# YuePanEdward/MULLS

Hardware: NVIDIA H100
Metric: scan-pair registrations/sec (120k-pt 64-beam) (higher is better)
Workload: dtype f32 geometry / f64 accumulation

## Files before the change

### mulls_b200/csrc/device_types.cuh

```cuda
#pragma once
#include <cstdint>
#include <cuda_runtime.h>

#include "../../include/mulls_b200/abi.h"
#include "search_core.cuh"

namespace mulls {

constexpr int kNumClasses = MULLS_NUM_CLASSES;
constexpr int kNumSegs = 2 * kNumClasses;
constexpr int kIterBlock = 128;
constexpr int kIngestBlock = 256;
constexpr int kTerms = 28;
constexpr int kMaxLevels = 12;
constexpr int kCoordBits = 12;
constexpr int kDedupMinSrc = 500;
constexpr unsigned kClaimFree = 0x7f7f7f7fu;
constexpr int kIterFlags = 256;

enum PairStatus : int { kRunning = 0, kNeedPosterior = 1, kDone = 2 };

struct ChunkDesc {
    uint32_t pair;
    uint32_t seg;
// ... 37 lines not shown
};

struct PairState {
    double T_total[16];
    double T_inc[16];
    double x[6];
    double cofactor[36];
    double info[36];
    double sigma2;
    double ibb[6];
    float thre;
    float confidence;
    float origin[3];
    float h0, inv_h0;
    int n_levels;
    int status, code, iter, iters_entered, final_buf;
    int source_feature_points_count;
    int n_src[kNumClasses];
    int n_src_g[kNumClasses];
    int n_src_g_next[kNumClasses];
    int n_tgt[kNumClasses];
    uint32_t n_corr[kNumClasses];
    uint32_t n_corr_last[kNumClasses];
    uint32_t seg_count[kNumSegs];
    uint32_t seg_start[kNumSegs];
    uint32_t hash_entries[kNumClasses];
    uint32_t hash_base[kNumClasses];
    uint32_t hash_mask[kNumClasses];
    int bb_src[6];
    int bb_tgt[6];
    uint64_t alg_bytes;
    int kl_keep[kNumSegs];
    uint32_t kl_rank[kNumSegs];
    uint64_t kl_prefix[kNumSegs];
    uint32_t kl_hist[kNumSegs][256];
};

struct LoopCtl {
    int it;
    int n_it_chunks;
    int n_pairs;
    int trace_on;
    int max_iter;
    unsigned solved;
    unsigned n_live[2];
    unsigned work[4];
};

struct DeviceArrays {
    const float4 *in_aos;
    uint64_t *keys_a, *keys_b;
    uint32_t *vals_a, *vals_b;
    float4 *tgt_pos, *tgt_nrm;
    float4 *src_pos[2], *src_nrm[2];
    int *src_prevj[2];
    float4 *src_cert[2];
    int *nn_idx;
    float *nn_d2;
    uint8_t *flags;
    int *corr_j;
    float *corr_w;
    unsigned *claim;
    HashEntry *hash;
    uint32_t hash_pool_entries;
    uint32_t *hash_used;
    uint32_t *blk_kept;
    double *partials;
    double *post_partials;
    PairConst *pc;
    PairState *ps;
    ChunkDesc *in_chunks;
    ChunkDesc *it_chunks;
    mulls_icp_trace *trace;
    int *xch_i32;
    double *xch_f64;
    LoopCtl *ctl;
    uint32_t *live_chunks;
    uint32_t live_stride;
    int *running;
    volatile int *h_running;
    volatile int *h_running_iter;
};

}
```

### mulls_b200/csrc/kernels_iterate.cuh

```cuda
#pragma once
#include <cooperative_groups.h>

#include "device_math.cuh"
#include "device_types.cuh"
#include "kernels_ingest.cuh"

namespace mulls {

__device__ __forceinline__ bool chunk_in_run(const DeviceArrays &A) { return blockIdx.x < (unsigned)A.ctl->n_it_chunks; }
__device__ __forceinline__ int loop_buf(const DeviceArrays &A, int buf) { return buf >= 0 ? buf : (A.ctl->it & 1); }
__device__ __forceinline__ mulls_icp_trace *trace_of(const DeviceArrays &A, uint32_t pair) {
    return (A.trace && A.ctl->trace_on) ? &A.trace[pair] : nullptr;
}

template <class Body>
__device__ __forceinline__ void for_each_live_chunk(const DeviceArrays &A, int parity, int which, Body body) {
    __shared__ uint32_t s_fetch;
    LoopCtl &ctl = *A.ctl;
    const uint32_t n = ctl.n_live[parity];
    const uint32_t *list = A.live_chunks + (size_t)parity * A.live_stride;
    for (;;) {
        __syncthreads();
        if (threadIdx.x == 0) s_fetch = atomicAdd(&ctl.work[which], 1u);
        __syncthreads();
// ... 26 lines not shown
}

constexpr int kStartLevel0 = 5;
constexpr int kLeafCount = 32;
constexpr int kDeferFromIter = 3;
constexpr float kReseedCells = 4.0f;

__device__ __forceinline__ GridView grid_of(const DeviceArrays &A, const PairConst &pc, const PairState &ps, int c) {
    GridView g;
    g.table = A.hash + ps.hash_base[c];
    g.mask = ps.hash_mask[c];
    g.pos = A.tgt_pos + pc.tgt_base[c];
    g.nrm = A.tgt_nrm + pc.tgt_base[c];
    g.ox = ps.origin[0], g.oy = ps.origin[1], g.oz = ps.origin[2];
    g.h0 = ps.h0, g.inv_h0 = ps.inv_h0;
    g.n_levels = ps.n_levels;
    g.leaf_count = kLeafCount;
    g.level_slack2 = 1.002001f;
    return g;
}

constexpr int kShootK = 10;

__device__ __forceinline__ void load_and_advance(DeviceArrays &A, const PairState &ps, int buf, uint32_t gi, bool valid,
                                                 float4 &p, float4 &n) {
    p = A.src_pos[buf][gi];
    n = A.src_nrm[buf][gi];
    if (valid && ps.iter > 0) {
        const double *t = ps.T_inc;
        const double px = p.x, py = p.y, pz = p.z, qx = n.x, qy = n.y, qz = n.z;
        p.x = (float)(t[0] * px + t[1] * py + t[2] * pz + t[3]);
        p.y = (float)(t[4] * px + t[5] * py + t[6] * pz + t[7]);
        p.z = (float)(t[8] * px + t[9] * py + t[10] * pz + t[11]);
        n.x = (float)(t[0] * qx + t[1] * qy + t[2] * qz);
        n.y = (float)(t[4] * qx + t[5] * qy + t[6] * qz);
        n.z = (float)(t[8] * qx + t[9] * qy + t[10] * qz);
        A.src_pos[buf][gi] = p;
        A.src_nrm[buf][gi] = n;
    }
}

__device__ __forceinline__ bool shoots(const PairConst &pc, int c) {
    return pc.normal_shooting && (c == MULLS_GROUND || c == MULLS_FACADE || c == MULLS_ROOF);
}

constexpr int kKeepFromIter = 3;

struct SearchFrame {
    GridView g;
    double max_dist_sqr;
    float r2_prune;
    bool defer;
};
__device__ __forceinline__ SearchFrame search_frame(const DeviceArrays &A, const PairConst &pc, const PairState &ps, int c) {
    SearchFrame f;
    f.g = grid_of(A, pc, ps, c);
    const float max_distance_f = 2.5f * ps.thre;
    f.max_dist_sqr = (double)max_distance_f * (double)max_distance_f;
    f.r2_prune = (float)f.max_dist_sqr * 1.0001f;
    f.defer = ps.iter >= kDeferFromIter;
    return f;
// ... 89 lines not shown
                need = true;
                const int pj = A.src_prevj[buf][gi];
                const float4 ce = A.src_cert[buf][gi];
                if (pj >= 0 && ce.w > 0.0f) {
                    const float4 q = __ldg(&f.g.pos[pj]);
                    const float d1 = flann_l2(p.x, p.y, p.z, q.x, q.y, q.z);
                    const float mv = flann_l2(p.x, p.y, p.z, ce.x, ce.y, ce.z);
                    if ((sqrtf(d1) + sqrtf(mv)) * 1.0001f + 3e-5f < ce.w * 0.9999f) {
                        search_finish(A, pc, c, gi, pj, d1, f.max_dist_sqr, n.w);
                        need = false;
                    }
                }
            }
        }
        const unsigned m = __ballot_sync(0xffffffffu, need);
        uint32_t base = 0;
        if (lane == 0 && m) base = atomicAdd(n_need, (uint32_t)__popc(m));
        base = __shfl_sync(0xffffffffu, base, 0);
        if (need) need_list[base + __popc(m & ((1u << lane) - 1u))] = (uint8_t)threadIdx.x;
    }
    __syncthreads();
    if (threadIdx.x < *n_need) {
        const uint32_t gi = pc.src_base[c] + cd.first + need_list[threadIdx.x];
        const float4 p = A.src_pos[buf][gi];
        search_one<WalkBounds>(A, pc, c, buf, gi, p, A.src_nrm[buf][gi].w, f, true);
    }
}

constexpr int kSearchBlocksPerSm = 10;
__device__ __forceinline__ int search_mode_of(int it) { return it >= kKeepFromIter ? 2 : (it == kKeepFromIter - 1 ? 1 : 0); }

template <int kMode>
__global__ void __launch_bounds__(kIterBlock, kSearchBlocksPerSm) k_search(DeviceArrays A, int buf, int it) {
    buf = loop_buf(A, buf);
    if (it < 0) it = A.ctl->it;
    if (blockIdx.x == 0 && threadIdx.x == 0) {
        LoopCtl &ctl = *A.ctl;
        ctl.work[1] = ctl.work[2] = ctl.work[3] = 0u;
        ctl.n_live[buf ^ 1] = 0u;
    }
    if (search_mode_of(it) != kMode) return;
    if (kMode == 2) {
        __shared__ uint8_t s_need[kIterBlock];
        __shared__ uint32_t s_n_need;
        for_each_live_chunk(A, buf, 0, [&](uint32_t chunk) { search_keep_chunk(A, buf, chunk, s_need, &s_n_need); });
    } else {
        const uint32_t n_units = (kIterBlock / 32) * A.ctl->n_live[buf];
// ... 36 lines not shown
    KnnList<kShootK> kl;
    knn_search(g, p.x, p.y, p.z, kStartLevel0, kShootK, kl);
    double min_dist = 1.7976931348623157e308;
    for (int t = 0; t < kl.n; ++t) {
        const float4 q = __ldg(&g.pos[kl.j[t]]);
        const float ptx = q.x - p.x, pty = q.y - p.y, ptz = q.z - p.z;
        const double Nx = n.x, Ny = n.y, Nz = n.z, Vx = ptx, Vy = pty, Vz = ptz;
        const double Cx = Ny * Vz - Nz * Vy, Cy = Nz * Vx - Nx * Vz, Cz = Nx * Vy - Ny * Vx;
        const double dist = Cx * Cx + (Cy * Cy + Cz * Cz);
        if (dist < min_dist) {
            min_dist = dist;
            sj = kl.j[t];
            sd2 = kl.d2[t];
        }
    }
    if (sj >= 0 && min_dist > (double)max_distance_f) sj = -1;
    if (sj >= 0) atomicMin(&A.claim[pc.tgt_base[c] + sj], (unsigned)__float_as_int(n.w));
    A.nn_idx[gi] = sj;
    A.nn_d2[gi] = sd2;
}
__global__ void __launch_bounds__(kIterBlock) k_search_shoot(DeviceArrays A, int buf) {
    buf = loop_buf(A, buf);
    for_each_live_chunk(A, buf, 3, [&](uint32_t chunk) { search_shoot_chunk(A, buf, chunk); });
}

__device__ __forceinline__ void resolve_body(DeviceArrays &A, int buf, uint32_t chunk) {
    const ChunkDesc cd = A.it_chunks[chunk];
    const PairConst &pc = A.pc[cd.pair];
    PairState &ps = A.ps[cd.pair];
    if (ps.status != kRunning) return;
    const int c = (int)cd.seg;
    const int ns = ps.n_src[c], nt = ps.n_tgt[c], nsg = ps.n_src_g[c];
    const uint32_t local = cd.first + threadIdx.x;
    const bool valid = (int)local < ns;
    const bool active = pc.used[c] && nsg >= 3 && nt >= 3;
    const bool dedup = active && nsg >= kDedupMinSrc;
    bool kept = false, pass = false;
    if (valid) {
        const uint32_t gi = pc.src_base[c] + local;
        const int j = A.nn_idx[gi];
        const bool matched = active && j >= 0;
        bool corr = matched;
        kept = true;
        if (dedup) {
            const float4 n = A.src_nrm[buf][gi];
            const bool winner = matched && A.claim[pc.tgt_base[c] + j] == (unsigned)__float_as_int(n.w);
            kept = winner;
            corr = winner;
        }
        if (corr) {
            const float d2 = A.nn_d2[gi];
            pass = d2 < ps.thre * ps.thre;
            if (pass && c != MULLS_VERTEX) {
                const float4 n = A.src_nrm[buf][gi];
                const float4 m = A.tgt_nrm[pc.tgt_base[c] + j];
                const double dot = (double)n.x * (double)m.x + (double)n.y * (double)m.y + (double)n.z * (double)m.z;
                const float cos_angle = (float)fabs(dot);
                if ((double)cos_angle < pc.cos_thre) pass = false;
            }
        }
        A.flags[gi] = (uint8_t)((kept ? 1 : 0) | (pass ? 2 : 0));
    }
    const unsigned kb = __ballot_sync(0xffffffffu, kept);
    const unsigned pb = __ballot_sync(0xffffffffu, pass);
    __shared__ unsigned s_kept[kIterBlock / 32], s_pass[kIterBlock / 32];
    if ((threadIdx.x & 31) == 0) {
        s_kept[threadIdx.x >> 5] = __popc(kb);
        s_pass[threadIdx.x >> 5] = __popc(pb);
    }
    __syncthreads();
    if (threadIdx.x == 0) {
        unsigned k = 0, p = 0;
        for (int w = 0; w < kIterBlock / 32; ++w) {
            k += s_kept[w];
            p += s_pass[w];
        }
        A.blk_kept[chunk] = k;
        if (p) atomicAdd(&ps.n_corr[c], p);
    }
}
__global__ void __launch_bounds__(kIterBlock) k_resolve(DeviceArrays A, int buf) {
    buf = loop_buf(A, buf);
    for_each_live_chunk(A, buf, 1, [&](uint32_t chunk) { resolve_body(A, buf, chunk); });
}

template <class Sink>
__device__ __forceinline__ void terms_pt2pl(const float4 p, const float pi, const float4 q, const float4 qn,
                                            float weight, int iter_num, bool dist_w, bool resid_w, bool inten_w,
                                            float window, Sink t, float &w_out) {
    const float px = p.x, py = p.y, pz = p.z, qx = q.x, qy = q.y, qz = q.z;
    const float ntx = qn.x, nty = qn.y, ntz = qn.z;
    float w = weight;
    const float a = ntz * py - nty * pz;
    const float b = ntx * pz - ntz * px;
    const float c = nty * px - ntx * py;
    const float d = ntx * qx + nty * qy + ntz * qz - ntx * px - nty * py - ntz * pz;
    const float dist = sqrtf(qx * qx + qy * qy + qz * qz);
    if (dist_w) w = w * weight_by_dist_adaptive(dist, iter_num);
    if (resid_w) w = w * weight_by_residual(fabsf(d), window);
    if (inten_w) w = w * weight_by_intensity((float)((double)pi + 0.0001), (float)((double)q.w + 0.0001));
    w_out = w;
    t[0] = w * ntx * ntx;
    t[1] = w * ntx * nty;
    t[2] = w * ntx * ntz;
// ... 242 lines not shown
                cof[6 * (3 + r) + cc] = J[r][0] * inv[6 * 3 + cc] + J[r][1] * inv[6 * 4 + cc] + J[r][2] * inv[6 * 5 + cc];
    }
    double *Tt = ps.T_inc;
    construct_trans_a(x, Tt);
    const double ts_norm = sqrt(Tt[3] * Tt[3] + Tt[7] * Tt[7] + Tt[11] * Tt[11]);
    const double rs_angle = fabs(rotation_angle(Tt));
    if (ts_norm > (double)pc.max_t || rs_angle > (double)pc.max_r) {
        ps.code = -1;
        ps.status = kDone;
        pair_left_running(A);
        return;
    }
    mat4_mul(Tt, ps.T_total, Tmp);
    for (int k = 0; k < 16; ++k) ps.T_total[k] = Tmp[k];
    if (i == pc.max_iter - 1 || (i > 2 && ts_norm < (double)pc.conv_t && rs_angle < (double)pc.conv_r)) {
        ps.status = kNeedPosterior;
        ps.final_buf = buf_written;
        pair_left_running(A);
        return;
    }
    ps.iter = i + 1;
}

__device__ __forceinline__ void accumulate_body(DeviceArrays &A, int buf, uint32_t chunk) {
    const ChunkDesc cd = A.it_chunks[chunk];
    const PairConst &pc = A.pc[cd.pair];
    PairState &ps = A.ps[cd.pair];
    if (ps.status != kRunning) return;
    const int c = (int)cd.seg;
    const int ns = ps.n_src[c];
    const uint32_t local = cd.first + threadIdx.x;
    const bool valid = (int)local < ns;
    const int lane = threadIdx.x & 31, warp = threadIdx.x >> 5;
    constexpr int kWarps = kIterBlock / 32;
    __shared__ double s_terms[27 * kIterBlock];
    __shared__ uint32_t s_off[kWarps + 1];
    __shared__ uint32_t s_base;

    if ((int)cd.first >= ns) return;
    uint32_t dst_local = 0;
    uint8_t fl = 0;
    uint32_t gi = 0;
    bool kept = false, pass = false;
    struct Column {
        double *base;
        __device__ __forceinline__ double &operator[](int k) const { return base[k * kIterBlock]; }
    } t = {s_terms + threadIdx.x};
    {
        uint32_t acc = 0;
        const uint32_t first_chunk = pc.class_chunk_begin[c];
        for (uint32_t b = first_chunk + threadIdx.x; b < chunk; b += kIterBlock) acc += A.blk_kept[b];
        for (int o = 16; o > 0; o >>= 1) acc += __shfl_xor_sync(0xffffffffu, acc, o);
        if (lane == 0) s_off[warp] = acc;
        __syncthreads();
        if (threadIdx.x == 0) {
            uint32_t tt = 0;
            for (int w = 0; w < kWarps; ++w) tt += s_off[w];
            s_base = tt;
        }
        __syncthreads();
    }
    if (valid) {
        gi = pc.src_base[c] + local;
        fl = A.flags[gi];
    }
    kept = (fl & 1) != 0, pass = (fl & 2) != 0;
    const unsigned kb = __ballot_sync(0xffffffffu, kept);
    if (lane == 0) s_off[warp] = __popc(kb);
    __syncthreads();
    if (threadIdx.x == 0) {
        uint32_t run = 0;
        for (int w = 0; w < kWarps; ++w) {
            const uint32_t tt = s_off[w];
            s_off[w] = run;
            run += tt;
        }
        s_off[kWarps] = run;
    }
    __syncthreads();
    dst_local = s_base + s_off[warp] + __popc(kb & ((1u << lane) - 1u));

    float w_store = 0.0f;
    int j = -1;
    float4 p = make_float4(0, 0, 0, 0), n = make_float4(0, 0, 0, 0);
    float d2 = 0.0f;
    if (valid) {
        p = A.src_pos[buf][gi];
        n = A.src_nrm[buf][gi];
        j = A.nn_idx[gi];
        d2 = A.nn_d2[gi];
        if (j >= 0) A.claim[pc.tgt_base[c] + j] = kClaimFree;
    }
    uint32_t n_corr[kNumClasses];
#pragma unroll
    for (int k = 0; k < kNumClasses; ++k) n_corr[k] = ps.n_corr[k];
    float ratio_unused;
    const bool few = too_few(pc, ps, n_corr, ratio_unused);
    if (pass && !few) {
        const float4 q = A.tgt_pos[pc.tgt_base[c] + j];
        const float4 qn = A.tgt_nrm[pc.tgt_base[c] + j];
        const int it = ps.iter;
        const bool resid_w = pc.w_residual && it > 2;
        const bool dist_w = pc.w_dist != 0, inten_w = pc.w_intensity != 0;
        if (c == MULLS_GROUND || c == MULLS_FACADE || c == MULLS_ROOF) {
            const float wc = (c == MULLS_FACADE) ? 1.0f : balanced_ground_weight(pc, n_corr);
            terms_pt2pl(p, p.w, q, qn, wc, it, dist_w, resid_w, inten_w, pc.win_pt2pl, t, w_store);
        } else if (c == MULLS_PILLAR || c == MULLS_BEAM) {
            terms_pt2li(p, p.w, q, qn, 1.0f, it, dist_w, resid_w, inten_w, pc.win_pt2li, t, w_store);
        } else {
            terms_pt2pt(p, p.w, q, 1.0f, it, dist_w, resid_w, inten_w, pc.win_pt2pt, t);
            w_store = d2;
        }
    } else {
#pragma unroll
        for (int k = 0; k < 27; ++k) t[k] = 0.0;
    }
    if (kept) {
        const uint32_t gd = pc.src_base[c] + dst_local;
        A.src_pos[buf ^ 1][gd] = p;
        A.src_nrm[buf ^ 1][gd] = n;
        A.src_prevj[buf ^ 1][gd] = j;
        A.src_cert[buf ^ 1][gd] = A.src_cert[buf][gi];
        A.corr_j[gd] = pass ? j : -1;
        A.corr_w[gd] = w_store;
    }
    __syncthreads();
#pragma unroll 1
    for (int k = warp; k < 27; k += kWarps) {
        const double *row = s_terms + k * kIterBlock;
        double v = ((row[lane] + row[lane + 32]) + row[lane + 64]) + row[lane + 96];
#pragma unroll
        for (int o = 16; o > 0; o >>= 1) v += __shfl_xor_sync(0xffffffffu, v, o);
        if (lane == 0) A.partials[(size_t)chunk * kTerms + k] = v;
    }
}
__global__ void __launch_bounds__(kIterBlock, 8) k_accumulate(DeviceArrays A, int buf) {
    buf = loop_buf(A, buf);
    if (blockIdx.x == 0 && threadIdx.x == 0) A.ctl->work[0] = 0u;
    for_each_live_chunk(A, buf, 2, [&](uint32_t chunk) { accumulate_body(A, buf, chunk); });
}

__device__ __forceinline__ void publish_live_chunks(const DeviceArrays &A, uint32_t pair, int next_parity) {
    __shared__ uint32_t s_base;
    __syncthreads();
    const PairConst &pc = A.pc[pair];
    const PairState &ps = A.ps[pair];
    if (ps.status != kRunning) return;
    uint32_t count[kNumClasses], total = 0;
#pragma unroll
    for (int c = 0; c < kNumClasses; ++c) {
        count[c] = (uint32_t)((ps.n_src[c] + kIterBlock - 1) / kIterBlock);
        total += count[c];
    }
    if (threadIdx.x == 0) s_base = atomicAdd(&A.ctl->n_live[next_parity], total);
    __syncthreads();
    uint32_t base = s_base;
#pragma unroll
    for (int c = 0; c < kNumClasses; ++c) {
        append_live_chunks(A, next_parity, pc.class_chunk_begin[c], count[c], base);
        base += count[c];
    }
}

__device__ __forceinline__ void solve_body(DeviceArrays &A, int buf, uint32_t pair) {
    const PairConst &pc = A.pc[pair];
    PairState &ps = A.ps[pair];
    if (ps.status != kRunning) return;
    const int lane = threadIdx.x & 31, warp = threadIdx.x >> 5, n_warps = blockDim.x >> 5;
    __shared__ double s_S[kNumClasses][kTerms];
    __shared__ double s_scratch[160];
    __shared__ int s_newn[kNumClasses];
    __shared__ uint32_t s_ncorr[kNumClasses];
    for (int cc = warp; cc < kNumClasses; cc += n_warps) {
        const uint32_t b0 = pc.class_chunk_begin[cc];
        const uint32_t live = (uint32_t)((ps.n_src[cc] + kIterBlock - 1) / kIterBlock);
        const uint32_t b1 = min(pc.class_chunk_begin[cc + 1], b0 + live);
        double a0 = 0.0, a1 = 0.0, a2 = 0.0, a3 = 0.0;
        if (lane < 27) {
            uint32_t b = b0;
            for (; b + 4 <= b1; b += 4) {
                a0 += A.partials[(size_t)(b + 0) * kTerms + lane];
                a1 += A.partials[(size_t)(b + 1) * kTerms + lane];
                a2 += A.partials[(size_t)(b + 2) * kTerms + lane];
                a3 += A.partials[(size_t)(b + 3) * kTerms + lane];
            }
            for (; b < b1; ++b) a0 += A.partials[(size_t)b * kTerms + lane];
        }
        if (lane < kTerms) s_S[cc][lane] = (lane < 27) ? ((a0 + a1) + (a2 + a3)) : 0.0;
        uint32_t acc = 0;
        for (uint32_t b = b0 + lane; b < b1; b += 32) acc += A.blk_kept[b];
        for (int o = 16; o > 0; o >>= 1) acc += __shfl_xor_sync(0xffffffffu, acc, o);
        if (lane == 0) {
            s_newn[cc] = (int)acc;
            s_ncorr[cc] = ps.n_corr[cc];
        }
    }
    __syncthreads();
    if (threadIdx.x == 0) {
        uint64_t srcpts = 0;
        for (int cc = 0; cc < kNumClasses; ++cc)
            if (pc.used[cc]) srcpts += (uint64_t)ps.n_src_g[cc];
        ps.alg_bytes += 28ull * srcpts;
        if (pc.sharded) {
            for (int cc = 0; cc < kNumClasses; ++cc) {
                ps.n_src[cc] = s_newn[cc];
                for (int k = 0; k < kTerms; ++k) A.xch_f64[cc * kTerms + k] = (k < 27) ? s_S[cc][k] : 0.0;
            }
        } else {
        mulls_icp_trace *tr = trace_of(A, pair);
        for (int cc = 0; cc < kNumClasses; ++cc) {
            ps.n_src[cc] = s_newn[cc];
            ps.n_src_g[cc] = s_newn[cc];
            ps.n_corr[cc] = s_ncorr[cc];
            if (tr && ps.iter < MULLS_MAX_TRACE_ITERS) tr->n_src[ps.iter][cc] = (uint32_t)ps.n_src[cc];
        }
        solve_and_advance(A, pair, &s_S[0][0], s_scratch, buf ^ 1);
        for (int cc = 0; cc < kNumClasses; ++cc) ps.n_corr[cc] = 0;
        }
    }
    if (!pc.sharded) publish_live_chunks(A, pair, buf ^ 1);
}
constexpr int kSolveThreads = kNumClasses * 32;
__global__ void __launch_bounds__(kSolveThreads) k_solve(DeviceArrays A, int buf, unsigned long long loop_handle) {
    LoopCtl &ctl = *A.ctl;
    if (blockIdx.x >= (unsigned)ctl.n_pairs) return;
    solve_body(A, loop_buf(A, buf), blockIdx.x);
    if (loop_handle == 0ull) return;
    __syncthreads();
    if (threadIdx.x == 0) {
        __threadfence();
        if (atomicAdd(&ctl.solved, 1u) == (unsigned)ctl.n_pairs - 1u) {
            ctl.solved = 0;
            const int it = ctl.it + 1;
            ctl.it = it;
            __threadfence();
            const bool again = *(volatile int *)A.running > 0 && it < ctl.max_iter;
            cudaGraphSetConditional((cudaGraphConditionalHandle)loop_handle, again ? 1u : 0u);
        }
    }
}

__global__ void __launch_bounds__(kIterBlock, 4) k_icp_loop(DeviceArrays A) {
    namespace cg = cooperative_groups;
    cg::grid_group grid = cg::this_grid();
    LoopCtl &ctl = *A.ctl;
    __shared__ uint8_t s_need[kIterBlock];
    __shared__ uint32_t s_n_need;
    const int n_pairs = ctl.n_pairs, max_iter = ctl.max_iter;
    for (int it = 0; it < max_iter; ++it) {
        const int buf = it & 1;
        const uint32_t *list = A.live_chunks + (size_t)buf * A.live_stride;
        const uint32_t n_live = ctl.n_live[buf];
        if (blockIdx.x == 0 && threadIdx.x == 0) ctl.n_live[buf ^ 1] = 0u;
        for (uint32_t w = blockIdx.x; w < n_live; w += gridDim.x) {
            const uint32_t chunk = list[w];
            if (it >= kKeepFromIter) search_keep_chunk(A, buf, chunk, s_need, &s_n_need);
            else if (it == kKeepFromIter - 1) search_quarter<WalkBounds>(A, buf, chunk, threadIdx.x >> 5, true);
            else search_quarter<NoBounds>(A, buf, chunk, threadIdx.x >> 5, false);
            __syncthreads();
        }
        grid.sync();
        for (uint32_t w = blockIdx.x; w < n_live; w += gridDim.x) {
            resolve_body(A, buf, list[w]);
            __syncthreads();
        }
        grid.sync();
        for (uint32_t w = blockIdx.x; w < n_live; w += gridDim.x) {
            accumulate_body(A, buf, list[w]);
            __syncthreads();
        }
        grid.sync();
        for (int pair = blockIdx.x; pair < n_pairs; pair += gridDim.x) {
            solve_body(A, buf, (uint32_t)pair);
            __syncthreads();
        }
        grid.sync();
        if (*(volatile int *)A.running <= 0) break;
    }
}

__global__ void k_shard_pack_setup(DeviceArrays A, int phase) {
    PairState &ps = A.ps[0];
    if (phase == 0) {
        for (int d = 0; d < 3; ++d) {
            A.xch_i32[d] = ps.bb_src[d];
            A.xch_i32[3 + d] = ~ps.bb_src[3 + d];
        }
    } else if (phase == 1) {
        for (int d = 0; d < 3; ++d) {
            ps.bb_src[d] = A.xch_i32[d];
            ps.bb_src[3 + d] = ~A.xch_i32[3 + d];
        }
    } else if (phase == 2) {
        for (int c = 0; c < kNumClasses; ++c) A.xch_i32[c] = ps.n_src[c];
    } else {
        const PairConst &pc = A.pc[0];
// ... 221 lines not shown
        const GridView g = grid_of(A, pc, ps, cls);
        const float px = xyz[3 * i], py = xyz[3 * i + 1], pz = xyz[3 * i + 2];
        const float rmax = 2.5f * pc.thre_unit;
        const float r2 = rmax * rmax * 1.0001f;
        NoStats st;
        walk_greedy_seed(g, px, py, pz, kStartLevel0, best_d2, best_j, st);
        nn_search_walk(g, px, py, pz, r2, kStartLevel0, false, best_d2, best_j, st);
        if (best_j >= 0 && !((double)best_d2 <= (double)rmax * (double)rmax)) best_j = -1;
        if (best_j >= 0) best_j = __float_as_int(__ldg(&g.nrm[best_j]).w);
    }
    out_idx[i] = best_j;
    out_d2[i] = best_j >= 0 ? best_d2 : INFINITY;
}

__global__ void k_state_init(DeviceArrays A, int n_pairs) {
    const int p = blockIdx.x * blockDim.x + threadIdx.x;
    if (p >= n_pairs) return;
    PairState &ps = A.ps[p];
    for (int d = 0; d < 3; ++d) {
        ps.bb_src[d] = ps.bb_tgt[d] = 0x7fffffff;
        ps.bb_src[3 + d] = ps.bb_tgt[3 + d] = (int)0x80000000;
    }
    for (int s = 0; s < kNumSegs; ++s) ps.seg_count[s] = ps.seg_start[s] = 0;
    for (int c = 0; c < kNumClasses; ++c) ps.hash_entries[c] = ps.n_corr[c] = 0;
    ps.status = kRunning;
    if (p == 0) {
        *A.running = n_pairs;
        *A.h_running = n_pairs;
    }
}

__global__ void k_collect(DeviceArrays A, int n_pairs, mulls_icp_result *out) {
    if (n_pairs < 0) n_pairs = A.ctl->n_pairs;
    const int p = blockIdx.x * blockDim.x + threadIdx.x;
    if (p >= n_pairs) return;
    const PairState &ps = A.ps[p];
    mulls_icp_result &r = out[p];
    for (int k = 0; k < 16; ++k) r.T[k] = ps.T_total[k];
    for (int k = 0; k < 36; ++k) r.info[k] = ps.info[k];
    r.sigma = (float)sqrt(ps.sigma2);
    r.confidence = ps.confidence;
    r.code = ps.code;
    r.iters = ps.iters_entered;
    for (int c = 0; c < kNumClasses; ++c) {
        r.n_corr[c] = ps.n_corr_last[c];
        r.n_src[c] = (uint32_t)ps.n_src_g[c];
    }
// ... 5 lines not shown
```

### mulls_b200/csrc/mulls_b200.cu

```cuda
#include <algorithm>
#include <atomic>
#include <memory>
#include <cmath>
#include <cstdio>
#include <chrono>
#include <cstring>
#include <string>
#include <vector>

#include <cub/device/device_radix_sort.cuh>
#include <cub/device/device_scan.cuh>

#include <dlfcn.h>
#include <mutex>

#include "device_types.cuh"
#include "host_pack.h"
#include "scan_io.h"
#include "kernels_ingest.cuh"
#include "kernels_iterate.cuh"
#include "kernels_pca.cuh"
#include "kernels_map.cuh"
#include "kernels_classify.cuh"
#include "kernels_ground.cuh"
// ... 75 lines not shown
    void *nccl_comm = nullptr;
    bool any_keep_less = false;
    bool grid_valid = false;
    int use_graph = 1;
    cudaGraph_t graph = nullptr;
    cudaGraphExec_t graph_exec = nullptr;
    int graph_key[2] = {-1, -1};
    LoopCtl *h_ctl = nullptr;
    int num_sms = 132;
    bool any_normal_shooting = false;
    bool any_undistort = false;
    int host_pack = 2;
    float4 *h_stage = nullptr;
    size_t h_stage_slots = 0;
    cudaEvent_t ev_begin = nullptr, ev_ingest = nullptr, ev_iter = nullptr, ev_end = nullptr, ev_h2d0 = nullptr;
    bool h2d_timed = false;
    float up_ms_pack = 0.f, up_ms_host = 0.f;
    std::vector<cudaEvent_t> ev_search;
    mulls_run_stats stats{};
    std::vector<void *> allocs;
    std::string err;
    mulls_ctx *twin = nullptr;
    int loop_kernel_blocks = 0;
    struct Pending {
        uint64_t launches = 0;
        int n_search_ev = 0;
        bool graphed = false, hooked = false, active = false;
        mulls_icp_trace *trace = nullptr;
        mulls_allreduce_fn hook = nullptr;
        void *user = nullptr;
    } pend;
    Scratch pca_buf;
    Scratch cls_buf;
    Scratch gf_buf, gf_cell_buf;
    Scratch vx_buf, ext_buf;
    Scratch sor_buf;
    Scratch raw_buf;
    const mulls_map *tree_map = nullptr;
    uint64_t tree_epoch = 0;
};

#define CK(call)                                                                                      \
    do {                                                                                              \
        cudaError_t e_ = (call);                                                                      \
        if (e_ != cudaSuccess) {                                                                      \
            ctx->err = std::string(#call) + ": " + cudaGetErrorString(e_);                            \
// ... 132 lines not shown
    ALLOC(A.tgt_pos, ct + kScanOverrun);
    ALLOC(A.tgt_nrm, ct);
    for (int b = 0; b < 2; ++b) {
        ALLOC(A.src_pos[b], cs);
        ALLOC(A.src_nrm[b], cs);
        ALLOC(A.src_prevj[b], cs);
        ALLOC(A.src_cert[b], cs);
    }
    ALLOC(A.nn_idx, cs);
    ALLOC(A.nn_d2, cs);
    ALLOC(A.flags, cs);
    ALLOC(A.corr_j, cs);
    ALLOC(A.corr_w, cs);
    ALLOC(A.claim, ct);
    {
        size_t pool = 12 * ct + 64 * max_pairs * kNumClasses;
        if (pool >= (1ull << 32)) pool = (1ull << 32) - 1;
        A.hash_pool_entries = (uint32_t)pool;
        ALLOC(A.hash, pool);
    }
    ALLOC(A.hash_used, 3);
    ALLOC(A.ctl, 1);
    ALLOC(A.blk_kept, ctx->cap_it_chunks);
    ALLOC(A.partials, ctx->cap_it_chunks * kTerms);
    ALLOC(A.post_partials, ctx->cap_it_chunks * 2);
    ALLOC(A.pc, max_pairs);
    ALLOC(A.ps, max_pairs);
    ALLOC(A.in_chunks, ctx->cap_in_chunks);
    ALLOC(A.it_chunks, ctx->cap_it_chunks);
    ALLOC(A.live_chunks, 2 * ctx->cap_it_chunks);
    A.live_stride = (uint32_t)ctx->cap_it_chunks;
    {
        int sms = 0;
        if (cudaDeviceGetAttribute(&sms, cudaDevAttrMultiProcessorCount, device) != cudaSuccess || sms <= 0) sms = 132;
        ctx->num_sms = sms;
    }
    ALLOC(ctx->d_results, max_pairs + ceil_div(max_pairs * sizeof(uint64_t), sizeof(mulls_icp_result)) + 1);
    ALLOC(ctx->d_trace, max_pairs);
    ALLOC(A.running, 1);
    ALLOC(A.xch_i32, 32);
    ALLOC(A.xch_f64, kNumClasses * kTerms + 8);
#undef ALLOC
    if ((e = cudaHostAlloc((void **)&ctx->h_running, (1 + kIterFlags) * sizeof(int), cudaHostAllocMapped)) != cudaSuccess)
        return fail("mapped flag", e);
    {
        int *dptr = nullptr;
        if ((e = cudaHostGetDevicePointer((void **)&dptr, ctx->h_running, 0)) != cudaSuccess) return fail("mapped flag", e);
        A.h_running = dptr;
        A.h_running_iter = dptr + 1;
    }
    ctx->ev_done.resize(MULLS_MAX_TRACE_ITERS);
    for (auto &ev : ctx->ev_done) cudaEventCreateWithFlags(&ev, cudaEventDisableTiming);
    A.trace = ctx->d_trace;
    if ((e = cudaMallocHost((void **)&ctx->h_results, max_pairs * (sizeof(mulls_icp_result) + sizeof(uint64_t)))) != cudaSuccess)
        return fail("pinned results", e);
    if ((e = cudaMallocHost((void **)&ctx->h_flags, 3 * sizeof(uint32_t))) != cudaSuccess) return fail("pinned flags", e);
    if ((e = cudaMallocHost((void **)&ctx->h_ctl, sizeof(LoopCtl))) != cudaSuccess) return fail("pinned control block", e);
    {
// ... 423 lines not shown
    } else {
        k_hash_layout<<<1, 32, 0, st>>>(A, np);
        ++launches;
    }
    return MULLS_OK;
}

static unsigned chunk_bucket(const mulls_ctx *ctx) {
    unsigned b = 1;
    while (b < (unsigned)ctx->h_it_chunks.size()) b <<= 1;
    return b;
}
static unsigned resident_grid(const mulls_ctx *ctx, int blocks_per_sm) {
    return std::min((unsigned)(ctx->num_sms * blocks_per_sm), chunk_bucket(ctx));
}
static void launch_search(mulls_ctx *ctx, cudaStream_t st, const DeviceArrays &A, int buf, int it) {
    const unsigned grid = resident_grid(ctx, kSearchBlocksPerSm);
    const int mode = it < 0 ? -1 : (it >= kKeepFromIter ? 2 : (it == kKeepFromIter - 1 ? 1 : 0));
    if (mode < 0 || mode == 0) k_search<0><<<grid, kIterBlock, 0, st>>>(A, buf, it);
    if (mode < 0 || mode == 1) k_search<1><<<grid, kIterBlock, 0, st>>>(A, buf, it);
    if (mode < 0 || mode == 2) k_search<2><<<grid, kIterBlock, 0, st>>>(A, buf, it);
}
constexpr int kShootBlocksPerSm = 8, kResolveBlocksPerSm = 16, kAccumulateBlocksPerSm = 8;
constexpr int kPollPause = 64;

static int build_iteration_graph(mulls_ctx *ctx) {
    const int key[2] = {(int)chunk_bucket(ctx), ctx->any_normal_shooting ? 1 : 0};
    if (ctx->graph_exec && std::memcmp(key, ctx->graph_key, sizeof(key)) == 0) return MULLS_OK;
    if (ctx->graph_exec) cudaGraphExecDestroy(ctx->graph_exec), ctx->graph_exec = nullptr;
    if (ctx->graph) cudaGraphDestroy(ctx->graph), ctx->graph = nullptr;
    cudaStream_t st = ctx->stream;
    DeviceArrays A = ctx->A;
    const unsigned cap_chunks = (unsigned)std::max<size_t>(ctx->cap_it_chunks, 1), cap_pairs = (unsigned)std::max<size_t>(ctx->max_pairs, 1);
    CK(cudaGraphCreate(&ctx->graph, 0));
    cudaGraphConditionalHandle handle;
    CK(cudaGraphConditionalHandleCreate(&handle, ctx->graph, 1, cudaGraphCondAssignDefault));
    cudaGraphNodeParams wp = {cudaGraphNodeTypeConditional};
    wp.conditional.handle = handle;
    wp.conditional.type = cudaGraphCondTypeWhile;
    wp.conditional.size = 1;
    cudaGraphNode_t while_node;
    CK(cudaGraphAddNode(&while_node, ctx->graph, nullptr, 0, &wp));
    cudaGraph_t body = wp.conditional.phGraph_out[0];
    CK(cudaStreamBeginCaptureToGraph(st, body, nullptr, nullptr, 0, cudaStreamCaptureModeThreadLocal));
    launch_search(ctx, st, A, -1, -1);
    if (ctx->any_normal_shooting)
        k_search_shoot<<<resident_grid(ctx, kShootBlocksPerSm), kIterBlock, 0, st>>>(A, -1);
    k_resolve<<<resident_grid(ctx, kResolveBlocksPerSm), kIterBlock, 0, st>>>(A, -1);
    k_accumulate<<<resident_grid(ctx, kAccumulateBlocksPerSm), kIterBlock, 0, st>>>(A, -1);
    k_solve<<<cap_pairs, kSolveThreads, 0, st>>>(A, -1, (unsigned long long)handle);
    CK(cudaStreamEndCapture(st, nullptr));
    CK(cudaStreamBeginCaptureToGraph(st, ctx->graph, &while_node, nullptr, 1, cudaStreamCaptureModeThreadLocal));
    k_posterior<<<std::min(cap_chunks, chunk_bucket(ctx)), kIterBlock, 0, st>>>(A);
    k_finalize<<<(unsigned)ceil_div(cap_pairs, 64), 64, 0, st>>>(A, -1);
    k_collect<<<(unsigned)ceil_div(cap_pairs, 128), 128, 0, st>>>(A, -1, ctx->d_results);
    CK(cudaStreamEndCapture(st, nullptr));
    CK(cudaGraphInstantiate(&ctx->graph_exec, ctx->graph, 0));
    std::memcpy(ctx->graph_key, key, sizeof(key));
    return MULLS_OK;
}

static int grow_hash_pool(mulls_ctx *ctx) {
    const uint32_t need = ctx->h_flags[2];
    DeviceArrays &A = ctx->A;
    if (need <= A.hash_pool_entries || need == 0xffffffffu) {
        ctx->err = "hash pool exhausted (the target clouds need " + std::to_string(need) + " grid entries)";
        return MULLS_E_CAPACITY;
    }
    HashEntry *fresh = nullptr;
    if (cudaMalloc(&fresh, (size_t)need * sizeof(HashEntry)) != cudaSuccess) {
        cudaGetLastError();
        ctx->err = "hash pool exhausted, and no device memory to grow it to " + std::to_string(need) + " entries";
        return MULLS_E_CAPACITY;
// ... 92 lines not shown
            launch_search(ctx, st, A, buf, it);
            if (ctx->any_normal_shooting) {
                k_search_shoot<<<resident_grid(ctx, kShootBlocksPerSm), kIterBlock, 0, st>>>(A, buf);
                ++launches;
            }
            CK(cudaEventRecord(ctx->ev_search[2 * it + 1], st));
            if (hook) {
                if (hook(user, A.claim, ctx->n_tgt_total, 1, 1, (void *)st) != 0) {
                    ctx->err = "all-reduce callback failed";
                    return MULLS_E_COMM;
                }
            }
            k_resolve<<<resident_grid(ctx, kResolveBlocksPerSm), kIterBlock, 0, st>>>(A, buf);
            if (hook) {
                k_shard_counts<<<1, kIterBlock, 0, st>>>(A, 0);
                if (hook(user, A.xch_i32, 2 * kNumClasses, 1, 0, (void *)st) != 0) {
                    ctx->err = "all-reduce callback failed";
                    return MULLS_E_COMM;
                }
                k_shard_counts<<<1, kIterBlock, 0, st>>>(A, 1);
                launches += 2;
            }
            k_accumulate<<<resident_grid(ctx, kAccumulateBlocksPerSm), kIterBlock, 0, st>>>(A, buf);
            k_solve<<<(unsigned)np, kSolveThreads, 0, st>>>(A, buf, 0ull);
            if (hook) {
                if (hook(user, A.xch_f64, kNumClasses * kTerms, 0, 0, (void *)st) != 0) {
                    ctx->err = "all-reduce callback failed";
                    return MULLS_E_COMM;
                }
                k_shard_solve<<<1, 32, 0, st>>>(A, buf, std::min(it, kIterFlags - 1));
                ++launches;
            }
            CK(cudaEventRecord(ctx->ev_done[it], st));
            launches += 4;
            n_search_ev = it + 1;
        }
        k_posterior<<<n_itc, kIterBlock, 0, st>>>(A);
        if (hook) {
            k_shard_post<<<1, 32, 0, st>>>(A, 0);
            if (hook(user, A.xch_f64, 2, 0, 0, (void *)st) != 0) {
                ctx->err = "all-reduce callback failed";
                return MULLS_E_COMM;
            }
            k_shard_post<<<1, 32, 0, st>>>(A, 1);
            launches += 3;
        } else {
            k_finalize<<<(unsigned)ceil_div(np, 64), 64, 0, st>>>(A, np);
// ... 1384 lines not shown
```

Measured before the change: 6178.

## Fuse transform into consumers, precompute kept offsets, stage solve partials in shared memory

Stops writing transformed source points back in load_and_advance and instead re-applies the incremental transform at each consumer (shoot, resolve, accumulate). Resolve's last block per class now runs a block-wide scan over per-chunk kept counts, replacing accumulate's per-block prefix sum and solve's kept sum. k_solve moves to 512 threads and stages partials through dynamic shared memory with vectorised loads. The src_cert copy is skipped when the search mode does not need it. The trade is extra recomputation of the transform, a last-block atomic/threadfence pattern, and more shared memory per solve block.

```diff
diff --git a/mulls_b200/csrc/device_types.cuh b/mulls_b200/csrc/device_types.cuh
--- a/mulls_b200/csrc/device_types.cuh
+++ b/mulls_b200/csrc/device_types.cuh
@@ -83,6 +83,8 @@
     int n_tgt[kNumClasses];
     uint32_t n_corr[kNumClasses];
     uint32_t n_corr_last[kNumClasses];
+    uint32_t kept_done[kNumClasses];
+    uint32_t n_kept[kNumClasses];
     uint32_t seg_count[kNumSegs];
     uint32_t seg_start[kNumSegs];
     uint32_t hash_entries[kNumClasses];
@@ -126,6 +128,7 @@
     uint32_t hash_pool_entries;
     uint32_t *hash_used;
     uint32_t *blk_kept;
+    uint32_t *blk_off;
     double *partials;
     double *post_partials;
     PairConst *pc;
diff --git a/mulls_b200/csrc/kernels_iterate.cuh b/mulls_b200/csrc/kernels_iterate.cuh
--- a/mulls_b200/csrc/kernels_iterate.cuh
+++ b/mulls_b200/csrc/kernels_iterate.cuh
@@ -72,21 +72,31 @@
 
 constexpr int kShootK = 10;
 
-__device__ __forceinline__ void load_and_advance(DeviceArrays &A, const PairState &ps, int buf, uint32_t gi, bool valid,
+__device__ __forceinline__ void advance_pos(const PairState &ps, float4 &p) {
+    if (ps.iter > 0) {
+        const double *t = ps.T_inc;
+        const double px = p.x, py = p.y, pz = p.z;
+        p.x = (float)(t[0] * px + t[1] * py + t[2] * pz + t[3]);
+        p.y = (float)(t[4] * px + t[5] * py + t[6] * pz + t[7]);
+        p.z = (float)(t[8] * px + t[9] * py + t[10] * pz + t[11]);
+    }
+}
+__device__ __forceinline__ void advance_nrm(const PairState &ps, float4 &n) {
+    if (ps.iter > 0) {
+        const double *t = ps.T_inc;
+        const double qx = n.x, qy = n.y, qz = n.z;
+        n.x = (float)(t[0] * qx + t[1] * qy + t[2] * qz);
+        n.y = (float)(t[4] * qx + t[5] * qy + t[6] * qz);
+        n.z = (float)(t[8] * qx + t[9] * qy + t[10] * qz);
+    }
+}
+__device__ __forceinline__ void load_and_advance(const DeviceArrays &A, const PairState &ps, int buf, uint32_t gi, bool valid,
                                                  float4 &p, float4 &n) {
     p = A.src_pos[buf][gi];
     n = A.src_nrm[buf][gi];
-    if (valid && ps.iter > 0) {
-        const double *t = ps.T_inc;
-        const double px = p.x, py = p.y, pz = p.z, qx = n.x, qy = n.y, qz = n.z;
-        p.x = (float)(t[0] * px + t[1] * py + t[2] * pz + t[3]);
-        p.y = (float)(t[4] * px + t[5] * py + t[6] * pz + t[7]);
-        p.z = (float)(t[8] * px + t[9] * py + t[10] * pz + t[11]);
-        n.x = (float)(t[0] * qx + t[1] * qy + t[2] * qz);
-        n.y = (float)(t[4] * qx + t[5] * qy + t[6] * qz);
-        n.z = (float)(t[8] * qx + t[9] * qy + t[10] * qz);
-        A.src_pos[buf][gi] = p;
-        A.src_nrm[buf][gi] = n;
+    if (valid) {
+        advance_pos(ps, p);
+        advance_nrm(ps, n);
     }
 }
 
@@ -222,7 +232,8 @@
     __syncthreads();
     if (threadIdx.x < *n_need) {
         const uint32_t gi = pc.src_base[c] + cd.first + need_list[threadIdx.x];
-        const float4 p = A.src_pos[buf][gi];
+        float4 p = A.src_pos[buf][gi];
+        advance_pos(ps, p);
         search_one<WalkBounds>(A, pc, c, buf, gi, p, A.src_nrm[buf][gi].w, f, true);
     }
 }
@@ -305,6 +316,44 @@
 __global__ void __launch_bounds__(kIterBlock) k_search_shoot(DeviceArrays A, int buf) {
     buf = loop_buf(A, buf);
     for_each_live_chunk(A, buf, 3, [&](uint32_t chunk) { search_shoot_chunk(A, buf, chunk); });
+}
+
+constexpr int kScanItems = 4;
+__device__ __forceinline__ uint32_t scan_kept_offsets(const uint32_t *blk_kept, uint32_t *blk_off, uint32_t b0, uint32_t n_chunks) {
+    __shared__ uint32_t s_warp[kIterBlock / 32];
+    const int lane = threadIdx.x & 31, warp = threadIdx.x >> 5;
+    uint32_t carry = 0;
+    for (uint32_t r0 = 0; r0 < n_chunks; r0 += kIterBlock * kScanItems) {
+        const uint32_t lo = r0 + threadIdx.x * kScanItems;
+        uint32_t v[kScanItems], s = 0;
+#pragma unroll
+        for (int k = 0; k < kScanItems; ++k) {
+            v[k] = (lo + k < n_chunks) ? __ldcg(&blk_kept[b0 + lo + k]) : 0u;
+            s += v[k];
+        }
+        uint32_t incl = s;
+#pragma unroll
+        for (int o = 1; o < 32; o <<= 1) {
+            const uint32_t u = __shfl_up_sync(0xffffffffu, incl, o);
+            if (lane >= o) incl += u;
+        }
+        if (lane == 31) s_warp[warp] = incl;
+        __syncthreads();
+        uint32_t run = carry + incl - s, total = 0;
+#pragma unroll
+        for (int w = 0; w < kIterBlock / 32; ++w) {
+            if (w < warp) run += s_warp[w];
+            total += s_warp[w];
+        }
+#pragma unroll
+        for (int k = 0; k < kScanItems; ++k) {
+            if (lo + k < n_chunks) blk_off[b0 + lo + k] = run;
+            run += v[k];
+        }
+        carry += total;
+        __syncthreads();
+    }
+    return carry;
 }
 
 __device__ __forceinline__ void resolve_body(DeviceArrays &A, int buf, uint32_t chunk) {
@@ -335,7 +384,8 @@
             const float d2 = A.nn_d2[gi];
             pass = d2 < ps.thre * ps.thre;
             if (pass && c != MULLS_VERTEX) {
-                const float4 n = A.src_nrm[buf][gi];
+                float4 n = A.src_nrm[buf][gi];
+                advance_nrm(ps, n);
                 const float4 m = A.tgt_nrm[pc.tgt_base[c] + j];
                 const double dot = (double)n.x * (double)m.x + (double)n.y * (double)m.y + (double)n.z * (double)m.z;
                 const float cos_angle = (float)fabs(dot);
@@ -352,6 +402,7 @@
         s_pass[threadIdx.x >> 5] = __popc(pb);
     }
     __syncthreads();
+    __shared__ bool s_last;
     if (threadIdx.x == 0) {
         unsigned k = 0, p = 0;
         for (int w = 0; w < kIterBlock / 32; ++w) {
@@ -360,9 +411,21 @@
         }
         A.blk_kept[chunk] = k;
         if (p) atomicAdd(&ps.n_corr[c], p);
-    }
-}
-__global__ void __launch_bounds__(kIterBlock) k_resolve(DeviceArrays A, int buf) {
+        __threadfence();
+        const uint32_t n_chunks = (uint32_t)((ns + kIterBlock - 1) / kIterBlock);
+        s_last = atomicAdd(&ps.kept_done[c], 1u) == n_chunks - 1u;
+    }
+    __syncthreads();
+    if (s_last) {
+        const uint32_t total = scan_kept_offsets(A.blk_kept, A.blk_off, pc.class_chunk_begin[c],
+                                                 (uint32_t)((ns + kIterBlock - 1) / kIterBlock));
+        if (threadIdx.x == 0) {
+            ps.n_kept[c] = total;
+            ps.kept_done[c] = 0u;
+        }
+    }
+}
+__global__ void __launch_bounds__(kIterBlock, 16) k_resolve(DeviceArrays A, int buf) {
     buf = loop_buf(A, buf);
     for_each_live_chunk(A, buf, 1, [&](uint32_t chunk) { resolve_body(A, buf, chunk); });
 }
@@ -651,6 +714,12 @@
     ps.iter = i + 1;
 }
 
+__device__ __forceinline__ double *term_matrix() {
+    __shared__ __align__(16) double s_terms[27 * kIterBlock];
+    return s_terms;
+}
+constexpr uint32_t kTermMatrixChunks = (27 * kIterBlock / kTerms) & ~3u;
+
 __device__ __forceinline__ void accumulate_body(DeviceArrays &A, int buf, uint32_t chunk) {
     const ChunkDesc cd = A.it_chunks[chunk];
     const PairConst &pc = A.pc[cd.pair];
@@ -662,9 +731,8 @@
     const bool valid = (int)local < ns;
     const int lane = threadIdx.x & 31, warp = threadIdx.x >> 5;
     constexpr int kWarps = kIterBlock / 32;
-    __shared__ double s_terms[27 * kIterBlock];
+    double *s_terms = term_matrix();
     __shared__ uint32_t s_off[kWarps + 1];
-    __shared__ uint32_t s_base;
 
     if ((int)cd.first >= ns) return;
     uint32_t dst_local = 0;
@@ -675,20 +743,7 @@
         double *base;
         __device__ __forceinline__ double &operator[](int k) const { return base[k * kIterBlock]; }
     } t = {s_terms + threadIdx.x};
-    {
-        uint32_t acc = 0;
-        const uint32_t first_chunk = pc.class_chunk_begin[c];
-        for (uint32_t b = first_chunk + threadIdx.x; b < chunk; b += kIterBlock) acc += A.blk_kept[b];
-        for (int o = 16; o > 0; o >>= 1) acc += __shfl_xor_sync(0xffffffffu, acc, o);
-        if (lane == 0) s_off[warp] = acc;
-        __syncthreads();
-        if (threadIdx.x == 0) {
-            uint32_t tt = 0;
-            for (int w = 0; w < kWarps; ++w) tt += s_off[w];
-            s_base = tt;
-        }
-        __syncthreads();
-    }
+    const uint32_t s_base = A.blk_off[chunk];
     if (valid) {
         gi = pc.src_base[c] + local;
         fl = A.flags[gi];
@@ -716,6 +771,8 @@
     if (valid) {
         p = A.src_pos[buf][gi];
         n = A.src_nrm[buf][gi];
+        advance_pos(ps, p);
+        advance_nrm(ps, n);
         j = A.nn_idx[gi];
         d2 = A.nn_d2[gi];
         if (j >= 0) A.claim[pc.tgt_base[c] + j] = kClaimFree;
@@ -749,7 +806,7 @@
         A.src_pos[buf ^ 1][gd] = p;
         A.src_nrm[buf ^ 1][gd] = n;
         A.src_prevj[buf ^ 1][gd] = j;
-        A.src_cert[buf ^ 1][gd] = A.src_cert[buf][gi];
+        if (search_mode_of(ps.iter) != 0) A.src_cert[buf ^ 1][gd] = A.src_cert[buf][gi];
         A.corr_j[gd] = pass ? j : -1;
         A.corr_w[gd] = w_store;
     }
@@ -791,7 +848,9 @@
     }
 }
 
-__device__ __forceinline__ void solve_body(DeviceArrays &A, int buf, uint32_t pair) {
+constexpr int kSolveSlots = 2;
+constexpr int kStageLoads = 8;
+__device__ __forceinline__ void solve_body(DeviceArrays &A, int buf, uint32_t pair, double *stage, uint32_t stage_chunks) {
     const PairConst &pc = A.pc[pair];
     PairState &ps = A.ps[pair];
     if (ps.status != kRunning) return;
@@ -800,27 +859,74 @@
     __shared__ double s_scratch[160];
     __shared__ int s_newn[kNumClasses];
     __shared__ uint32_t s_ncorr[kNumClasses];
-    for (int cc = warp; cc < kNumClasses; cc += n_warps) {
-        const uint32_t b0 = pc.class_chunk_begin[cc];
-        const uint32_t live = (uint32_t)((ps.n_src[cc] + kIterBlock - 1) / kIterBlock);
-        const uint32_t b1 = min(pc.class_chunk_begin[cc + 1], b0 + live);
-        double a0 = 0.0, a1 = 0.0, a2 = 0.0, a3 = 0.0;
-        if (lane < 27) {
-            uint32_t b = b0;
-            for (; b + 4 <= b1; b += 4) {
-                a0 += A.partials[(size_t)(b + 0) * kTerms + lane];
-                a1 += A.partials[(size_t)(b + 1) * kTerms + lane];
-                a2 += A.partials[(size_t)(b + 2) * kTerms + lane];
-                a3 += A.partials[(size_t)(b + 3) * kTerms + lane];
+    uint32_t b0[kNumClasses], live[kNumClasses], start[kNumClasses + 1];
+    start[0] = 0;
+#pragma unroll
+    for (int cc = 0; cc < kNumClasses; ++cc) {
+        b0[cc] = pc.class_chunk_begin[cc];
+        live[cc] = (uint32_t)((ps.n_src[cc] + kIterBlock - 1) / kIterBlock);
+        start[cc + 1] = start[cc] + ((live[cc] + 3u) & ~3u);
+    }
+    double acc[kSolveSlots][4];
+#pragma unroll
+    for (int s = 0; s < kSolveSlots; ++s) acc[s][0] = acc[s][1] = acc[s][2] = acc[s][3] = 0.0;
+    for (uint32_t t0 = 0; t0 < start[kNumClasses]; t0 += stage_chunks) {
+        const uint32_t tn = min(stage_chunks, start[kNumClasses] - t0);
+        __syncthreads();
+#pragma unroll
+        for (int cc = 0; cc < kNumClasses; ++cc) {
+            const uint32_t lo = max(start[cc], t0), hi = min(start[cc] + live[cc], t0 + tn);
+            if (lo >= hi) continue;
+            const double2 *src = reinterpret_cast<const double2 *>(A.partials + (size_t)(b0[cc] + lo - start[cc]) * kTerms);
+            double2 *dst = reinterpret_cast<double2 *>(stage + (size_t)(lo - t0) * kTerms);
+            const uint32_t n2 = (hi - lo) * (kTerms / 2);
+            for (uint32_t e0 = threadIdx.x; e0 < n2; e0 += kStageLoads * blockDim.x) {
+                double2 v[kStageLoads];
+#pragma unroll
+                for (int u = 0; u < kStageLoads; ++u) {
+                    const uint32_t e = e0 + u * blockDim.x;
+                    if (e < n2) v[u] = __ldcg(src + e);
+                }
+#pragma unroll
+                for (int u = 0; u < kStageLoads; ++u) {
+                    const uint32_t e = e0 + u * blockDim.x;
+                    if (e < n2) dst[e] = v[u];
+                }
             }
-            for (; b < b1; ++b) a0 += A.partials[(size_t)b * kTerms + lane];
-        }
-        if (lane < kTerms) s_S[cc][lane] = (lane < 27) ? ((a0 + a1) + (a2 + a3)) : 0.0;
-        uint32_t acc = 0;
-        for (uint32_t b = b0 + lane; b < b1; b += 32) acc += A.blk_kept[b];
-        for (int o = 16; o > 0; o >>= 1) acc += __shfl_xor_sync(0xffffffffu, acc, o);
+        }
+        __syncthreads();
+#pragma unroll
+        for (int s = 0; s < kSolveSlots; ++s) {
+            const int cc = warp + s * n_warps;
+            if (cc >= kNumClasses || lane >= 27) continue;
+            uint32_t cs = 0, cl = 0;
+#pragma unroll
+            for (int q = 0; q < kNumClasses; ++q)
+                if (q == cc) cs = start[q], cl = live[q];
+            if (cs + cl <= t0 || cs >= t0 + tn) continue;
+            const uint32_t r_first = max(cs, t0) - cs, rh = min(cs + cl, t0 + tn) - cs, n4 = cl & ~3u;
+            const double *v = stage + (size_t)(cs + r_first - t0) * kTerms + lane;
+            double a0 = acc[s][0], a1 = acc[s][1], a2 = acc[s][2], a3 = acc[s][3];
+            uint32_t r = r_first;
+#pragma unroll 4
+            for (; r + 4 <= min(rh, n4); r += 4) {
+                const double *g = v + (size_t)(r - r_first) * kTerms;
+                a0 += g[0 * kTerms];
+                a1 += g[1 * kTerms];
+                a2 += g[2 * kTerms];
+                a3 += g[3 * kTerms];
+            }
+            for (; r < rh; ++r) a0 += v[(size_t)(r - r_first) * kTerms];
+            acc[s][0] = a0, acc[s][1] = a1, acc[s][2] = a2, acc[s][3] = a3;
+        }
+    }
+#pragma unroll
+    for (int s = 0; s < kSolveSlots; ++s) {
+        const int cc = warp + s * n_warps;
+        if (cc >= kNumClasses) continue;
+        if (lane < kTerms) s_S[cc][lane] = (lane < 27) ? ((acc[s][0] + acc[s][1]) + (acc[s][2] + acc[s][3])) : 0.0;
         if (lane == 0) {
-            s_newn[cc] = (int)acc;
+            s_newn[cc] = ps.n_src[cc] > 0 ? (int)ps.n_kept[cc] : 0;
             s_ncorr[cc] = ps.n_corr[cc];
         }
     }
@@ -849,11 +955,13 @@
     }
     if (!pc.sharded) publish_live_chunks(A, pair, buf ^ 1);
 }
-constexpr int kSolveThreads = kNumClasses * 32;
-__global__ void __launch_bounds__(kSolveThreads) k_solve(DeviceArrays A, int buf, unsigned long long loop_handle) {
+constexpr int kSolveThreads = 512;
+__global__ void __launch_bounds__(kSolveThreads) k_solve(DeviceArrays A, int buf, unsigned long long loop_handle,
+                                                         uint32_t stage_chunks) {
+    extern __shared__ __align__(16) double s_stage[];
     LoopCtl &ctl = *A.ctl;
     if (blockIdx.x >= (unsigned)ctl.n_pairs) return;
-    solve_body(A, loop_buf(A, buf), blockIdx.x);
+    solve_body(A, loop_buf(A, buf), blockIdx.x, s_stage, stage_chunks);
     if (loop_handle == 0ull) return;
     __syncthreads();
     if (threadIdx.x == 0) {
@@ -900,7 +1008,7 @@
         }
         grid.sync();
         for (int pair = blockIdx.x; pair < n_pairs; pair += gridDim.x) {
-            solve_body(A, buf, (uint32_t)pair);
+            solve_body(A, buf, (uint32_t)pair, term_matrix(), kTermMatrixChunks);
             __syncthreads();
         }
         grid.sync();
@@ -1168,7 +1276,7 @@
         ps.bb_src[3 + d] = ps.bb_tgt[3 + d] = (int)0x80000000;
     }
     for (int s = 0; s < kNumSegs; ++s) ps.seg_count[s] = ps.seg_start[s] = 0;
-    for (int c = 0; c < kNumClasses; ++c) ps.hash_entries[c] = ps.n_corr[c] = 0;
+    for (int c = 0; c < kNumClasses; ++c) ps.hash_entries[c] = ps.n_corr[c] = ps.kept_done[c] = 0;
     ps.status = kRunning;
     if (p == 0) {
         *A.running = n_pairs;
diff --git a/mulls_b200/csrc/mulls_b200.cu b/mulls_b200/csrc/mulls_b200.cu
--- a/mulls_b200/csrc/mulls_b200.cu
+++ b/mulls_b200/csrc/mulls_b200.cu
@@ -121,6 +121,7 @@
     std::string err;
     mulls_ctx *twin = nullptr;
     int loop_kernel_blocks = 0;
+    uint32_t solve_stage_chunks = 4;
     struct Pending {
         uint64_t launches = 0;
         int n_search_ev = 0;
@@ -299,6 +300,7 @@
     ALLOC(A.hash_used, 3);
     ALLOC(A.ctl, 1);
     ALLOC(A.blk_kept, ctx->cap_it_chunks);
+    ALLOC(A.blk_off, ctx->cap_it_chunks);
     ALLOC(A.partials, ctx->cap_it_chunks * kTerms);
     ALLOC(A.post_partials, ctx->cap_it_chunks * 2);
     ALLOC(A.pc, max_pairs);
@@ -311,6 +313,14 @@
         int sms = 0;
         if (cudaDeviceGetAttribute(&sms, cudaDevAttrMultiProcessorCount, device) != cudaSuccess || sms <= 0) sms = 132;
         ctx->num_sms = sms;
+    }
+    {
+        constexpr size_t kSolveStageMax = 768;
+        const size_t need = ceil_div(max_src_pts, kIterBlock) + 4 * kNumClasses;
+        ctx->solve_stage_chunks = (uint32_t)((std::min(need, kSolveStageMax) + 3) & ~size_t(3));
+        const int bytes = (int)(kSolveStageMax * kTerms * sizeof(double));
+        if ((e = cudaFuncSetAttribute(k_solve, cudaFuncAttributeMaxDynamicSharedMemorySize, bytes)) != cudaSuccess)
+            return fail("k_solve shared memory", e);
     }
     ALLOC(ctx->d_results, max_pairs + ceil_div(max_pairs * sizeof(uint64_t), sizeof(mulls_icp_result)) + 1);
     ALLOC(ctx->d_trace, max_pairs);
@@ -780,6 +790,7 @@
     if (mode < 0 || mode == 2) k_search<2><<<grid, kIterBlock, 0, st>>>(A, buf, it);
 }
 constexpr int kShootBlocksPerSm = 8, kResolveBlocksPerSm = 16, kAccumulateBlocksPerSm = 8;
+static size_t solve_smem(const mulls_ctx *ctx) { return (size_t)ctx->solve_stage_chunks * kTerms * sizeof(double); }
 constexpr int kPollPause = 64;
 
 static int build_iteration_graph(mulls_ctx *ctx) {
@@ -806,7 +817,7 @@
         k_search_shoot<<<resident_grid(ctx, kShootBlocksPerSm), kIterBlock, 0, st>>>(A, -1);
     k_resolve<<<resident_grid(ctx, kResolveBlocksPerSm), kIterBlock, 0, st>>>(A, -1);
     k_accumulate<<<resident_grid(ctx, kAccumulateBlocksPerSm), kIterBlock, 0, st>>>(A, -1);
-    k_solve<<<cap_pairs, kSolveThreads, 0, st>>>(A, -1, (unsigned long long)handle);
+    k_solve<<<cap_pairs, kSolveThreads, solve_smem(ctx), st>>>(A, -1, (unsigned long long)handle, ctx->solve_stage_chunks);
     CK(cudaStreamEndCapture(st, nullptr));
     CK(cudaStreamBeginCaptureToGraph(st, ctx->graph, &while_node, nullptr, 1, cudaStreamCaptureModeThreadLocal));
     k_posterior<<<std::min(cap_chunks, chunk_bucket(ctx)), kIterBlock, 0, st>>>(A);
@@ -945,7 +956,7 @@
                 launches += 2;
             }
             k_accumulate<<<resident_grid(ctx, kAccumulateBlocksPerSm), kIterBlock, 0, st>>>(A, buf);
-            k_solve<<<(unsigned)np, kSolveThreads, 0, st>>>(A, buf, 0ull);
+            k_solve<<<(unsigned)np, kSolveThreads, solve_smem(ctx), st>>>(A, buf, 0ull, ctx->solve_stage_chunks);
             if (hook) {
                 if (hook(user, A.xch_f64, kNumClasses * kTerms, 0, 0, (void *)st) != 0) {
                     ctx->err = "all-reduce callback failed";
```

Result: no change. 6185 (median of 6 runs) (+0.1%).
